# hbb1/2d-gaussian-splatting

Measured on AMD Instinct MI355X. Metric: train iters/sec (full iteration: rasterizer fwd+bwd, L1+SSIM, normal+dist regularisers, Adam) + fwd Msplats/s @1080p, higher is better.
Workload: dtype f32; 1 GPU; garden: trained synthetic capture, 5400000 initial points -> 2136144 surfels after 2500 iterations of the reference schedule, 32 views of 1600x1060; steady-state iteration, every loss term on; P=2136144, image=1600x1060, n_pass=6, tiles=6700

## Files before the change

2d-gaussian-splatting_amd/csrc/surfel_api.hip:

```cpp
#include <cstring>
#include <mutex>
#include <string>
#include <vector>

#include <hip/hip_runtime.h>

#include "../../include/surfel_debug.h"
#include "surfel_common.h"
#include "surfel_kernels.h"
#include "train_kernels.h"

using namespace surfel;

namespace {

const char* kStageNames[] = {"preprocess_fwd", "depth_sort_scan", "emit_instances", "tile_sort", "tile_ranges", "blend_fwd",
                             "zero_grec", "blend_bwd", "preprocess_bwd", "knn", "tile_depth_sort"};
enum Stage { ST_PRE = 0, ST_SCAN, ST_EMIT, ST_SORT, ST_RANGES, ST_BLEND, ST_ZERO, ST_BBWD, ST_PBWD, ST_KNN, ST_TSORT, ST_COUNT };
static_assert(sizeof(kStageNames) / sizeof(kStageNames[0]) == ST_COUNT, "one name per stage");

struct CapEntry {
    int W = 0, H = 0; int64_t maxR = -1; unsigned frames = 0; int uniform_streak = 0; int boost = 0; unsigned last_overflow = 0;
    int slot() const; void begin_frame(); int64_t capacity(int end_bit) const; void record_count(int64_t R, bool overflowed);
};
// ... 43 lines not shown
    template <typename T> T* take(size_t count) {
        off = align_up(off);
        T* p = base ? reinterpret_cast<T*>(base + off) : nullptr;
        off += count * sizeof(T);
        return p;
    }
    size_t size() const { return align_up(off); }
};

struct GeomState {
    float* rec; float* depths; uint32_t* tiles_touched; uint8_t* clamped;
    uint32_t *dkey_a, *dkey_b, *ord_a, *ord_b;
    uint32_t* offsets;
    uint32_t* rects;
    float* shjac;
    char* temp;
    static GeomState carve(void* base, int P, size_t temp_bytes, size_t* total) {
        Carver c(base); GeomState g;
        g.rec = c.take<float>((size_t)P * REC_F);
        g.depths = c.take<float>(P);
        g.tiles_touched = c.take<uint32_t>(P);
        g.clamped = c.take<uint8_t>(P);
        g.dkey_a = c.take<uint32_t>(P); g.dkey_b = c.take<uint32_t>(P);
        g.ord_a = c.take<uint32_t>(P); g.ord_b = c.take<uint32_t>(P);
        g.offsets = c.take<uint32_t>(P);
        g.rects = c.take<uint32_t>(P);
        g.shjac = c.take<float>((size_t)9 * P);
        g.temp = c.take<char>(temp_bytes);
        if (total) *total = c.size();
        return g;
    }
};

struct BinState {
    uint32_t* point_list; uint32_t* vals_alt; uint32_t* keys_a; uint32_t* keys_b; char* sort_temp;
    float4* strm_rec = nullptr; uint32_t* strm_mask = nullptr;
    static bool wants_stream(size_t R) { return g_opt_stream != 0 && R > 0 && (long long)R <= STRM_MAX_R; }
    static BinState carve(void* base, size_t R, size_t sort_bytes, size_t* total, bool stream = false) {
        Carver c(base); BinState b;
        b.point_list = c.take<uint32_t>(R);
        b.vals_alt = c.take<uint32_t>(R);
        b.keys_a = c.take<uint32_t>(R);
// ... 204 lines not shown
    tm.begin(); launch_tile_depth_sort(pa.gx * pa.gy, maxR, img.ranges, bin.point_list, geom.dkey_a, bin.vals_alt, bin.keys_a, bin.keys_b, fused_ranges, s);
    STAGE_END(tm, ST_TSORT);
    return 0;
}

int64_t bin_exact(const PreprocessArgs& pa, int end_bit, int per_tile, int64_t R, const GeomState& geom, BinState* bin,
                  const ImgState& img, const uint32_t* hR, hipEvent_t evR, bool stream, surfel_alloc_fn binning_alloc, void* binning_user,
                  StageTimer& tm, hipStream_t s) {
    if (per_tile < 0 && R < 0) {
        HIP_TRY(hipEventSynchronize(evR));
        per_tile = per_tile_pays(pinned_total(hR, false), pa.gx, pa.gy);
    }
    tm.begin();
    const uint32_t* order = geom.ord_a;
    if (!per_tile) {
        const int which = radix_sort_pairs_u32(geom.dkey_a, geom.ord_a, geom.dkey_b, geom.ord_b, (size_t)pa.P, 0, 32, geom.temp, s, true);
        if (which < 0) return fail(SURFEL_E_LIMIT, "too many surfels for the depth sort");
        order = which ? geom.ord_b : geom.ord_a;
    }
    launch_scan_gather(geom.tiles_touched, order, pa.pack_tiles, geom.offsets, (size_t)pa.P, pa.zero_b, s);
    STAGE_END(tm, ST_SCAN);
    if (R < 0) {
        HIP_TRY(hipEventSynchronize(evR));
        R = pinned_total(hR, false);
    }
    if (int e = alloc_bin((size_t)R, radix_sort_scratch_bytes((size_t)R), stream, binning_alloc, binning_user, bin)) return e;
    if (R == 0) return 0;
    const bool odd = radix_sort_result_buffer((size_t)R, 0, end_bit) == 1;
    uint32_t* va = odd ? bin->vals_alt : bin->point_list;
    uint32_t* vb = odd ? bin->point_list : bin->vals_alt;
    tm.begin();
    launch_emit_instances(pa.P, geom.rec, geom.rects, order, pa.pack_tiles ? ((1u << PACK_ID_BITS) - 1u) : 0xffffffffu, geom.offsets, bin->keys_a, va, pa.gx,
                          reinterpret_cast<uint32_t*>(bin->sort_temp), (uint32_t)radix_sort_head_words((size_t)R), s);
    STAGE_END(tm, ST_EMIT);
    tm.begin();
    const int wk = radix_sort_pairs_u32(bin->keys_a, va, bin->keys_b, vb, (size_t)R, 0, end_bit, bin->sort_temp, s, true);
    if (wk < 0) return fail(SURFEL_E_LIMIT, "too many tile instances for the tile sort");
    STAGE_END(tm, ST_SORT);
    tm.begin(); launch_tile_ranges(R, wk ? bin->keys_b : bin->keys_a, img.ranges, s); STAGE_END(tm, ST_RANGES);
    if (per_tile) {
        tm.begin(); launch_tile_depth_sort(pa.gx * pa.gy, R, img.ranges, bin->point_list, geom.dkey_a, bin->vals_alt, bin->keys_a, bin->keys_b, false, s);
        STAGE_END(tm, ST_TSORT);
    }
    return R;
}

int blend(CapEntry* ce, int W, int H, int gx, int gy, const ImgState& img, const void* img_base, const BinState& bin, const float* rec,
          const float* background, float* out_color, float* out_others, int avg_list, bool jac, int tile_order, StageTimer& tm, hipStream_t s) {
    run_tile_order(ce, img.ranges, gx, gy, img.tile_map, img.total + 2 * R_SLOTS + 1, tile_order, s);
    BlendFwdArgs ba{};
    ba.W = W; ba.H = H; ba.gx = gx; ba.gy = gy;
    ba.ranges = img.ranges; ba.point_list = bin.point_list; ba.rec = rec; ba.bg = background;
    ba.out_color = out_color; ba.out_others = out_others; ba.final_T = img.final_T; ba.n_contrib = img.n_contrib;
    ba.tile_map = img.tile_map; ba.map_flag = img.total + 2 * R_SLOTS + 1; ba.map_len = tile_map_len(gx, gy);
// ... 189 lines not shown
        GeomState::carve(nullptr, P, temp_bytes, &geom_bytes);
        void* geom_base = geom_alloc(geom_user, geom_bytes);
        if (!geom_base) return fail(SURFEL_E_ALLOC, "geometry buffer allocation failed");
        geom = GeomState::carve(geom_base, P, temp_bytes, nullptr);

        PreprocessArgs pa{};
        pa.P = P; pa.D = D; pa.M = M; pa.W = width; pa.H = height; pa.gx = gx; pa.gy = gy; pa.scale_modifier = scale_modifier;
        pa.cull = opt_cull;
        pa.pack_tiles = P < (1 << PACK_ID_BITS) ? 1 : 0;
        pa.means3D = means3D; pa.opacities = opacities; pa.scales = scales; pa.rotations = rotations;
        pa.transMat_precomp = transMat_precomp; pa.colors_precomp = colors_precomp; pa.shs = shs;
        pa.viewmatrix = viewmatrix; pa.projmatrix = projmatrix; pa.campos = cam_pos;
        pa.rec = geom.rec; pa.depths = geom.depths; pa.depth_keys = geom.dkey_a; pa.ident = geom.ord_a; pa.radii = radii;
        pa.tiles_touched = geom.tiles_touched; pa.clamped = geom.clamped; pa.total_instances = img.total; pa.rects = geom.rects;
        pa.shjac = jac ? geom.shjac : nullptr;
        pa.zero_a = reinterpret_cast<uint32_t*>(geom.temp); pa.zero_a_words = (uint32_t)radix_sort_head_words((size_t)P);
        pa.zero_b = reinterpret_cast<uint32_t*>(geom.temp + psort_bytes); pa.zero_b_words = (uint32_t)scan_scratch_words((size_t)P);

        const int end_bit = higher_msb((uint32_t)(gx * gy));
        int per_tile = opt_tile_sort == 2 ? 1 : (opt_tile_sort == 0 ? 0 : -1);
        if (per_tile < 0 && g_th.last_R >= 0 && g_th.last_W == width && g_th.last_H == height) per_tile = per_tile_pays(g_th.last_R, gx, gy);
        const int64_t cap = (opt_capacity && per_tile == 1 && debug != 1) ? ce->capacity(end_bit) : 0;
        if (cap > 0) {
            if (int e = alloc_bin((size_t)cap, capacity_sort_scratch_bytes((size_t)cap, end_bit), opt_stream, binning_alloc, binning_user, &bin)) return e;
            pa.zero_c = reinterpret_cast<uint32_t*>(bin.sort_temp); pa.zero_c_words = (uint32_t)bin_emit_head_words();
            pa.block_totals = geom.offsets;
        }
        tm.begin(); launch_preprocess_fwd(pa, s); STAGE_END(tm, ST_PRE);
        uint32_t* hR = pinned_u32();
        hipEvent_t evR = r_event();
// ... 51 lines not shown
    hipStream_t s = static_cast<hipStream_t>(stream);
    if (P == 0) return 0;
    if (!scratch_alloc || !geom_buffer || !binning_buffer || !image_buffer) return fail(SURFEL_E_INVALID, "buffer / allocator is NULL");
    if (!dL_dout_color || !dL_dout_others || !dL_dmeans2D || !dL_dopacity || !dL_dcolors || !dL_dmeans3D)
        return fail(SURFEL_E_INVALID, "gradient pointer is NULL");
    if (transMat_precomp && !dL_dtransMat) return fail(SURFEL_E_INVALID, "dL_dtransMat is NULL but transMat_precomp was given");
    if (!transMat_precomp && (!dL_dscales || !dL_drots || !scales || !rotations)) return fail(SURFEL_E_INVALID, "scale/rotation pointers are NULL");
    const int gx = (width + TILE - 1) / TILE, gy = (height + TILE - 1) / TILE;

    GeomState geom = GeomState::carve(const_cast<void*>(geom_buffer), P, 0, nullptr);
    BinState bin = BinState::carve(const_cast<void*>(binning_buffer), (size_t)R, 0, nullptr);
    ImgState img = ImgState::carve(const_cast<void*>(image_buffer), width, height, nullptr);

    const size_t grec_bytes = align_up((size_t)(R > 0 ? R : 1) * GREC_F * sizeof(float));
    const size_t cut_bytes = align_up((size_t)gx * gy * sizeof(uint2));
    float* grec = static_cast<float*>(scratch_alloc(scratch_user, grec_bytes + cut_bytes + (size_t)P));
    if (!grec) return fail(SURFEL_E_ALLOC, "gradient record allocation failed");
    const bool use_cut = (debug_in & SURFEL_OPT_TILE_CUTS) ? true : ((debug_in & SURFEL_OPT_ZERO_RECORDS) ? false : R >= ((int64_t)1 << 21));
    uint2* cut = use_cut ? reinterpret_cast<uint2*>(reinterpret_cast<char*>(grec) + grec_bytes) : nullptr;
    uint8_t* has_rec = use_cut ? reinterpret_cast<uint8_t*>(grec) + grec_bytes + cut_bytes : nullptr;
    if (has_rec) HIP_TRY(hipMemsetAsync(has_rec, 0, (size_t)P, s));
    StageTimer tm(debug, s);

    BlendBwdArgs bb{};
    bb.W = width; bb.H = height; bb.gx = gx; bb.gy = gy;
    bb.ranges = img.ranges; bb.point_list = bin.point_list; bb.rec = geom.rec; bb.bg = background;
    bb.final_T = img.final_T; bb.n_contrib = img.n_contrib; bb.dL_dpix = dL_dout_color; bb.dL_dothers = dL_dout_others;
    bb.tile_map = img.tile_map; bb.map_flag = img.total + 2 * R_SLOTS + 1; bb.map_len = tile_map_len(gx, gy);
    bb.grec = grec; bb.cut = cut; bb.has_rec = has_rec; bb.depths = geom.depths; bb.variant = opt_variant; bb.stats = g_blend_stats; bb.walk_word = img.total + 2 * R_SLOTS + 2;
    bool have_jac = false;
    {
        const float4* srec = nullptr; const uint32_t* smask = nullptr;
        const bool found = stream_lookup(binning_buffer, image_buffer, &srec, &smask, &have_jac);
        if (found && !(debug_in & SURFEL_OPT_BWD_GATHER) && g_opt_stream) { bb.strm_rec = srec; bb.strm_mask = smask; }
    }
    bb.n_dev = img.total + 2 * R_SLOTS; bb.n_cap = (uint32_t)(R < 0xffffffffll ? R : 0xffffffffll);
// ... 57 lines not shown
```

2d-gaussian-splatting_amd/csrc/surfel_kernels.h:

```cpp
#pragma once
#include <hip/hip_runtime.h>
#include <stdint.h>

namespace surfel {

struct PreprocessArgs {
    int P, D, M, W, H, gx, gy;
    int cull;
    int pack_tiles;
    float scale_modifier;
    const float* means3D; const float* opacities; const float* scales; const float* rotations;
    const float* transMat_precomp; const float* colors_precomp; const float* shs;
    const float* viewmatrix; const float* projmatrix; const float* campos;
    float* rec; float* depths; uint32_t* depth_keys; uint32_t* ident; int* radii; uint32_t* tiles_touched; uint8_t* clamped;
    uint32_t* rects;
    float* shjac;
    uint32_t* total_instances;
    uint32_t* block_totals;
    uint32_t* zero_a; uint32_t zero_a_words;
    uint32_t* zero_b; uint32_t zero_b_words;
    uint32_t* zero_c; uint32_t zero_c_words;
};

struct BlendFwdArgs {
    int W, H, gx, gy;
    const uint2* ranges; const uint32_t* point_list; const float* rec; const float* bg;
    float* out_color; float* out_others; float* final_T; uint32_t* n_contrib;
    const int* tile_map; const uint32_t* map_flag; int map_len;
    unsigned long long* stats;
    int avg_list;
    float4* strm_rec; uint32_t* strm_mask;
    const uint32_t* totals; uint32_t* walk_word;
};

struct BlendBwdArgs {
    int W, H, gx, gy;
// ... 37 lines not shown
void launch_tile_order(const uint2* ranges, int gx, int gy, int* map, uint32_t* map_flag , int force, uint32_t* verdict, hipStream_t s);
void launch_blend_fwd(const BlendFwdArgs& a, hipStream_t s);
bool launch_blend_fwd_writes_stream(const BlendFwdArgs& a);
void set_fwd_pipe(int v);
void launch_mark_visible(int P, const float* means3D, const float* vm, uint8_t* present, hipStream_t s);
void launch_blend_bwd(const BlendBwdArgs& a, hipStream_t s);
void launch_blend_bwd_scan(const BlendBwdArgs& a, hipStream_t s);
void launch_preprocess_bwd(const PreprocessBwdArgs& a, hipStream_t s);
void launch_colour_gradients(const PreprocessBwdArgs& a, hipStream_t s);
void launch_knn(int P, const float* points, float* out, void* scratch, size_t scratch_bytes, hipStream_t s);
size_t knn_scratch_bytes(int P);
size_t radix_sort_scratch_bytes(size_t n);
void set_large_sort_impl(int v);
int radix_sort_passes(size_t n, int begin_bit, int end_bit);
int radix_sort_result_buffer(size_t n, int begin_bit, int end_bit);
int radix_sort_pairs_u32(uint32_t* keys_a, uint32_t* vals_a, uint32_t* keys_b, uint32_t* vals_b, size_t n, int begin_bit, int end_bit,
                         void* scratch, hipStream_t s, bool head_zeroed = false);
size_t radix_sort_head_words(size_t n);
size_t scan_scratch_words(size_t n);
void launch_tile_depth_sort(int ntiles, int64_t R, uint2* ranges, uint32_t* point_list, const uint32_t* depth_keys, uint32_t* tmp_ids,
                            uint32_t* tmp_keys, uint32_t* tmp_rank, bool decode, hipStream_t s);
void launch_scan_gather(const uint32_t* vals, const uint32_t* order, int packed, uint32_t* out, size_t n, void* zeroed_scratch, hipStream_t s);
bool capacity_binning_ok(size_t cap, int end_bit);
size_t capacity_sort_scratch_bytes(size_t cap, int end_bit);
size_t bin_emit_head_words();
void launch_bin_emit(int P, const uint32_t* tiles_touched, const uint32_t* rects, const uint32_t* block_totals, float* rec, uint32_t* keys, uint32_t* vals,
                     int gx, size_t cap, void* sort_scratch , int end_bit, uint32_t* n_out, uint32_t* n_host ,
                     hipStream_t s);
int radix_sort_pairs_u32_devn(uint32_t* keys_a, uint32_t* vals_a, uint32_t* keys_b, uint32_t* vals_b, size_t cap, int end_bit, const uint32_t* n_dev,
                              void* scratch, uint2* ranges, hipStream_t s);
void launch_tile_ranges_devn(size_t cap, const uint32_t* n_dev, const uint32_t* keys, uint2* ranges, hipStream_t s);

// ... 2 lines not shown
```

2d-gaussian-splatting_amd/csrc/surfel_preprocess.hip:

```cpp
#include "surfel_common.h"
#include "surfel_kernels.h"

namespace surfel {


__device__ __constant__ float SH_C0 = 0.28209479177387814f;
__device__ __constant__ float SH_C1 = 0.4886025119029199f;
__device__ __constant__ float SH_C2[5] = {1.0925484305920792f, -1.0925484305920792f, 0.31539156525252005f,
                                          -1.0925484305920792f, 0.5462742152960396f};
__device__ __constant__ float SH_C3[7] = {-0.5900435899266435f, 2.890611442640554f, -0.4570457994644658f,
                                          0.3731763325901154f, -0.4570457994644658f, 1.445305721320277f,
                                          -0.5900435899266435f};

__device__ __forceinline__ void sh_basis_gradient(int D, float x, float y, float z, float (&Bx)[16], float (&By)[16], float (&Bz)[16]) {
#pragma unroll
    for (int k = 0; k < 16; k++) { Bx[k] = 0.f; By[k] = 0.f; Bz[k] = 0.f; }
    if (D > 0) {
        By[1] = -SH_C1; Bz[2] = SH_C1; Bx[3] = -SH_C1;
        if (D > 1) {
            const float xx = x * x, yy = y * y, zz = z * z, xy = x * y, yz = y * z, xz = x * z;
            Bx[4] = SH_C2[0] * y; By[4] = SH_C2[0] * x;
            By[5] = SH_C2[1] * z; Bz[5] = SH_C2[1] * y;
            Bx[6] = SH_C2[2] * -2.f * x; By[6] = SH_C2[2] * -2.f * y; Bz[6] = SH_C2[2] * 4.f * z;
            Bx[7] = SH_C2[3] * z; Bz[7] = SH_C2[3] * x;
// ... 259 lines not shown
        const int wave = threadIdx.x >> 6, lane = threadIdx.x & 63;
        const int first = blockIdx.x * 256 + wave * 64;
        const int npieces = 12 * min(64, a.P - first);
        const float4* __restrict__ src = reinterpret_cast<const float4*>(a.shs) + (size_t)first * 12;
        const unsigned base = __builtin_amdgcn_readfirstlane(lds_offset(&s_sh[wave][0]));
#pragma unroll
        for (int v = 0; v < 12; v++) {
            const int p = v * 64 + lane;
            if (p < npieces) dma16(src + p, base + (unsigned)v * 1024u);
        }
        sh_lds = &s_sh[wave][lane * 12];
    }
    for (uint32_t w = (uint32_t)i; w < a.zero_a_words; w += gridDim.x * blockDim.x) a.zero_a[w] = 0u;
    for (uint32_t w = (uint32_t)i; w < a.zero_b_words; w += gridDim.x * blockDim.x) a.zero_b[w] = 0u;
    for (uint32_t w = (uint32_t)i; w < a.zero_c_words; w += gridDim.x * blockDim.x) a.zero_c[w] = 0u;
    uint32_t tiles = i < a.P ? preprocess_one(a, i, sh_lds) : 0u;
    const uint32_t vis = (uint32_t)__popcll(__ballot(tiles != 0u));
#pragma unroll
    for (int o = 32; o > 0; o >>= 1) tiles += __shfl_xor(tiles, o);
    if ((threadIdx.x & 63) == 0) { s_tot[threadIdx.x >> 6] = tiles; s_vis[threadIdx.x >> 6] = vis; }
    __syncthreads();
    if (threadIdx.x == 0) {
        const uint32_t t = s_tot[0] + s_tot[1] + s_tot[2] + s_tot[3];
        if (a.block_totals) a.block_totals[blockIdx.x] = t;
        if (t) {
            atomicAdd(a.total_instances + (blockIdx.x % R_SLOTS), t);
            atomicAdd(a.total_instances + R_SLOTS + (blockIdx.x % R_SLOTS), s_vis[0] + s_vis[1] + s_vis[2] + s_vis[3]);
        }
    }
}
// ... 649 lines not shown
```

2d-gaussian-splatting_amd/csrc/surfel_sort.hip:

```cpp
#include <hip/hip_runtime.h>
#include <stdint.h>

#include <cstring>
#include <rocprim/device/device_radix_sort.hpp>

#include "surfel_common.h"
#include "surfel_kernels.h"

namespace surfel {

constexpr size_t RS_ONESWEEP_MAX_ITEMS = (size_t)1 << 20;
constexpr size_t g_onesweep_max = RS_ONESWEEP_MAX_ITEMS;
int g_large_sort_impl = 2;
void set_large_sort_impl(int v) { g_large_sort_impl = v < 0 ? 0 : (v > 3 ? 2 : v); }
static inline bool use_rocprim(size_t n, int begin_bit, int end_bit) {
    if (begin_bit != 0) return false;
    if (g_large_sort_impl == 3) return true;
    if (n <= g_onesweep_max) return false;
    if (g_large_sort_impl != 2) return g_large_sort_impl == 1;
    return n > ((size_t)1 << 25);
}
static size_t rocprim_sort_temp_bytes(size_t n) {
    thread_local size_t last_n = 0, last_bytes = 0;
    if (n == last_n && last_bytes) return last_bytes;
// ... 2 lines not shown
    (void)rocprim::radix_sort_pairs(nullptr, bytes, nul, nul, nul, nul, n, 0u, 32u, (hipStream_t)0);
    last_n = n; last_bytes = bytes;
    return bytes;
}

constexpr int RS_THREADS = 256;
constexpr int RS_IPT = 8;
constexpr int RS_TILE = RS_THREADS * RS_IPT;
static inline bool rs_onesweep(size_t n) { return n <= g_onesweep_max; }
constexpr int RS_BITS = 8;
constexpr int RS_RADIX = 1 << RS_BITS;
constexpr int RS_MAX_PASSES = 4;
constexpr uint32_t ST_AGG = 1u << 30, ST_PREFIX = 2u << 30, ST_VALUE = (1u << 30) - 1u;

constexpr size_t RS_HEAD_WORDS = RS_MAX_PASSES * RS_RADIX + 64;

static inline uint32_t rs_nblocks(size_t n) { return (uint32_t)((n + RS_TILE - 1) / RS_TILE); }

size_t radix_sort_scratch_bytes(size_t n) {
    if (!rs_onesweep(n)) {
        const size_t own = ((size_t)RS_RADIX * rs_nblocks(n) + RS_RADIX) * sizeof(uint32_t) + 256;
        const size_t rp = rocprim_sort_temp_bytes(n) + 256;
        return own > rp ? own : rp;
    }
    const size_t own = (RS_HEAD_WORDS + (size_t)RS_MAX_PASSES * rs_nblocks(n) * RS_RADIX) * sizeof(uint32_t) + 256;
    const size_t rp = g_large_sort_impl == 3 ? rocprim_sort_temp_bytes(n) + 256 : 0;
    return own > rp ? own : rp;
}
int radix_sort_passes(size_t, int begin_bit, int end_bit) { return (end_bit - begin_bit + RS_BITS - 1) / RS_BITS; }
int radix_sort_result_buffer(size_t n, int begin_bit, int end_bit) {
    if (n == 0 || end_bit <= begin_bit) return 0;
    if (use_rocprim(n, begin_bit, end_bit)) return 1;
    return radix_sort_passes(n, begin_bit, end_bit) & 1;
}
size_t radix_sort_head_bytes() { return RS_HEAD_WORDS * sizeof(uint32_t); }

// ... 60 lines not shown
        __syncthreads();
        uint32_t woff = 0;
        for (int w = 0; w < wave; w++) woff += s_w[w];
        const uint32_t carry = s_carry;
        if (i < nblocks) row[i] = carry + woff + x - v;
        __syncthreads();
        if (threadIdx.x == RS_THREADS - 1) s_carry = carry + woff + x;
        __syncthreads();
    }
    if (threadIdx.x == 0) total[blockIdx.x] = s_carry;
}

constexpr int FT_THREADS = 1024, FT_IPT = 4, FT_TILE = FT_THREADS * FT_IPT, FT_WAVES = FT_THREADS / 64;
constexpr int FT_LB = 32;
static inline uint32_t ft_nblocks(size_t n) { return (uint32_t)((n + FT_TILE - 1) / FT_TILE); }

template <bool LOOKBACK, int IPT>
__global__ void __launch_bounds__(FT_THREADS) os_pass_fat_kernel(const uint32_t* __restrict__ keys, const uint32_t* __restrict__ vals,
                                                                 uint32_t* __restrict__ keys_out, uint32_t* __restrict__ vals_out, uint32_t n,
                                                                 int shift, uint32_t mask, const uint32_t* __restrict__ ghist,
                                                                 uint32_t* __restrict__ status, uint32_t* __restrict__ ticket,
                                                                 const uint32_t* __restrict__ n_dev, int hstride, uint2* __restrict__ ranges,
                                                                 uint32_t nblocks) {
    __shared__ uint32_t s_cnt[FT_WAVES][RS_RADIX];
    constexpr int TILE_ITEMS = FT_THREADS * IPT;
    __shared__ uint2 s_item[TILE_ITEMS];
    __shared__ uint32_t s_gbase[RS_RADIX];
    __shared__ uint32_t s_w[4][2];
    __shared__ uint32_t s_tile;
    const int lane = threadIdx.x & 63, wave = threadIdx.x >> 6;
    const uint32_t d_t = threadIdx.x;
    if (LOOKBACK && threadIdx.x == 0) s_tile = atomicAdd(ticket, 1u);
    for (int i = threadIdx.x; i < FT_WAVES * RS_RADIX; i += FT_THREADS) (&s_cnt[0][0])[i] = 0u;
    __syncthreads();
    const uint32_t tile = LOOKBACK ? s_tile : blockIdx.x;
    if (n_dev) n = min(n, *n_dev);
    if (tile * (uint32_t)TILE_ITEMS >= n) return;
    const uint32_t wbase = tile * (uint32_t)TILE_ITEMS + wave * (64 * IPT);
    uint32_t k[IPT], v[IPT], rank[IPT];
#pragma unroll
    for (int it = 0; it < IPT; it++) {
        const uint32_t e = wbase + it * 64 + lane;
        const bool valid = e < n;
        k[it] = valid ? keys[e] : 0xffffffffu;
// ... 74 lines not shown
    for (int it = 0; it < IPT; it++) {
        const uint32_t e = wbase + it * 64 + lane;
        if (e < n) {
            const uint32_t d = (k[it] >> shift) & mask;
            s_item[s_cnt[wave][d] + rank[it]] = make_uint2(k[it], v[it]);
        }
    }
    __syncthreads();
    const uint32_t items = min((uint32_t)TILE_ITEMS, n - tile * (uint32_t)TILE_ITEMS);
#pragma unroll
    for (int it = 0; it < IPT; it++) {
        const uint32_t q = (uint32_t)it * FT_THREADS + threadIdx.x;
        if (q < items) {
            const uint2 kv = s_item[q];
            const uint32_t dst = s_gbase[(kv.x >> shift) & mask] + q;
            keys_out[dst] = kv.x;
            vals_out[dst] = kv.y;
            if (ranges) {
                const bool first = q == 0u || s_item[q - 1].x != kv.x;
                const bool last = q + 1u == items || s_item[q + 1].x != kv.x;
                if (first) atomicMax(&ranges[kv.x].x, ~dst);
                if (last) atomicMax(&ranges[kv.x].y, dst + 1u);
            }
        }
    }
}

size_t radix_sort_head_words(size_t n) { return rs_onesweep(n) ? RS_HEAD_WORDS : 0; }

constexpr int SC_IPT = 8, SC_TILE = RS_THREADS * SC_IPT;
size_t scan_scratch_words(size_t n) { return 64 + (n + SC_TILE - 1) / SC_TILE; }

__global__ void __launch_bounds__(RS_THREADS) scan_gather_kernel(const uint32_t* __restrict__ vals, const uint32_t* __restrict__ order, int packed,
                                                                 uint32_t* __restrict__ out, uint32_t n, uint32_t* __restrict__ scratch) {
    __shared__ uint32_t s_w[4];
    __shared__ uint32_t s_tile, s_excl;
    uint32_t* ticket = scratch;
    uint32_t* status = scratch + 64;
    const int lane = threadIdx.x & 63, wave = threadIdx.x >> 6;
    if (threadIdx.x == 0) s_tile = atomicAdd(ticket, 1u);
    __syncthreads();
    const uint32_t tile = s_tile;
    const uint32_t base = tile * SC_TILE + threadIdx.x * SC_IPT;
    uint32_t v[SC_IPT], sum = 0;
#pragma unroll
    for (int i = 0; i < SC_IPT; i++) {
        const uint32_t e = base + i;
        uint32_t t = 0u;
        if (e < n) {
            const uint32_t ov = order[e];
            if (packed) { t = ov >> PACK_ID_BITS; if (t == PACK_TILES_MAX) t = vals[ov & ((1u << PACK_ID_BITS) - 1u)]; }
            else t = vals[ov];
        }
        v[i] = t;
        sum += v[i];
    }
    uint32_t x = sum;
#pragma unroll
    for (int o = 1; o < 64; o <<= 1) { const uint32_t y = __shfl_up(x, o); if (lane >= o) x += y; }
    if (lane == 63) s_w[wave] = x;
    __syncthreads();
    uint32_t woff = 0;
    for (int w = 0; w < wave; w++) woff += s_w[w];
    const uint32_t agg = s_w[0] + s_w[1] + s_w[2] + s_w[3];
    if (wave == 0) {
        uint32_t excl = 0;
        if (tile == 0) {
            if (lane == 0) st_agent(status, agg | ST_PREFIX);
        } else {
            if (lane == 0) st_agent(status + tile, agg | ST_AGG);
            int p = (int)tile - 1;
            for (;;) {
                const int idx = p - lane;
                const uint32_t sw = idx >= 0 ? ld_agent(status + idx) : ST_PREFIX;
                const unsigned long long ready = __ballot((sw >> 30) != 0u);
                const unsigned long long pref = __ballot((sw & ST_PREFIX) != 0u);
                const int nready = ready == ~0ull ? 64 : __builtin_ctzll(~ready);
                const int firstp = pref ? __builtin_ctzll(pref) : 64;
                const int take = min(nready, firstp + 1);
// ... 8 lines not shown
            if (lane == 0) st_agent(status + tile, (excl + agg) | ST_PREFIX);
        }
        if (lane == 0) s_excl = excl;
    }
    __syncthreads();
    uint32_t run = s_excl + woff + x - sum;
#pragma unroll
    for (int i = 0; i < SC_IPT; i++) {
        run += v[i];
        if (base + i < n) out[base + i] = run;
    }
}

void launch_scan_gather(const uint32_t* vals, const uint32_t* order, int packed, uint32_t* out, size_t n, void* zeroed_scratch, hipStream_t s) {
    if (n == 0) return;
    hipLaunchKernelGGL(scan_gather_kernel, dim3((unsigned)((n + SC_TILE - 1) / SC_TILE)), dim3(RS_THREADS), 0, s, vals, order, packed, out, (uint32_t)n,
                       static_cast<uint32_t*>(zeroed_scratch));
}


template <int E>
__device__ __forceinline__ void tile_sort_regs(uint32_t n, uint32_t* __restrict__ pl, const uint32_t* __restrict__ depth_keys,
                                               unsigned long long* __restrict__ s, uint32_t tid) {
    unsigned long long v[E];
#pragma unroll
    for (int e = 0; e < E; e++) {
        const uint32_t idx = (uint32_t)e * RS_THREADS + tid;
        v[e] = ~0ull;
        if (idx < n) { const uint32_t id = pl[idx]; v[e] = ((unsigned long long)depth_keys[id] << 32) | id; }
    }
#pragma unroll
// ... 82 lines not shown
    for (uint32_t i = tid; i < n; i += RS_THREADS) pl[rank[i]] = ids[i];
}

void launch_tile_depth_sort(int ntiles, int64_t R, uint2* ranges, uint32_t* point_list, const uint32_t* depth_keys, uint32_t* tmp_ids,
                            uint32_t* tmp_keys, uint32_t* tmp_rank, bool decode, hipStream_t st) {
    if (ntiles <= 0) return;
    if (R <= (int64_t)256 * ntiles)
        hipLaunchKernelGGL(tile_depth_sort_kernel<2048>, dim3(ntiles), dim3(RS_THREADS), 0, st, ranges, point_list, depth_keys, tmp_ids, tmp_keys,
                           tmp_rank, decode ? 1 : 0);
    else
        hipLaunchKernelGGL(tile_depth_sort_kernel<4096>, dim3(ntiles), dim3(RS_THREADS), 0, st, ranges, point_list, depth_keys, tmp_ids, tmp_keys,
                           tmp_rank, decode ? 1 : 0);
}

int radix_sort_pairs_u32(uint32_t* keys_a, uint32_t* vals_a, uint32_t* keys_b, uint32_t* vals_b, size_t n, int begin_bit, int end_bit,
                         void* scratch, hipStream_t s, bool head_zeroed) {
    if (n == 0 || end_bit <= begin_bit) return 0;
    if (n >= ST_VALUE) return -1;
    const uint32_t nblocks = rs_nblocks(n);
    const int passes = radix_sort_passes(n, begin_bit, end_bit);
    if (passes > RS_MAX_PASSES) return -1;
    int cur = 0;
    if (use_rocprim(n, begin_bit, end_bit)) {
        size_t bytes = rocprim_sort_temp_bytes(n);
        if (rocprim::radix_sort_pairs(scratch, bytes, keys_a, keys_b, vals_a, vals_b, n, (unsigned)begin_bit, (unsigned)end_bit, s) != hipSuccess) return -1;
        return 1;
    }
    if (!rs_onesweep(n)) {
        uint32_t* hist = static_cast<uint32_t*>(scratch);
        uint32_t* total = hist + (size_t)RS_RADIX * nblocks;
        for (int p = 0; p < passes; p++) {
            const int bit = begin_bit + p * RS_BITS;
            const int nb = end_bit - bit < RS_BITS ? end_bit - bit : RS_BITS;
            const uint32_t mask = (1u << nb) - 1u;
            const uint32_t* kin = cur ? keys_b : keys_a; const uint32_t* vin = cur ? vals_b : vals_a;
            uint32_t* kout = cur ? keys_a : keys_b; uint32_t* vout = cur ? vals_a : vals_b;
            const uint32_t fb = ft_nblocks(n);
            hipLaunchKernelGGL(rs_hist_fat_kernel<FT_IPT>, dim3(fb), dim3(FTH_THREADS), 0, s, kin, (uint32_t)n, bit, mask, hist, fb);
            hipLaunchKernelGGL(rs_scan_kernel, dim3(RS_RADIX), dim3(RS_THREADS), 0, s, hist, fb, total);
            hipLaunchKernelGGL((os_pass_fat_kernel<false, FT_IPT>), dim3(fb), dim3(FT_THREADS), 0, s, kin, vin, kout, vout, (uint32_t)n, bit, mask, total, hist,
                               (uint32_t*)nullptr, (const uint32_t*)nullptr, 1, (uint2*)nullptr, fb);
            cur ^= 1;
        }
        return cur;
    }
    uint32_t* ghist = static_cast<uint32_t*>(scratch);
    uint32_t* ticket = ghist + RS_MAX_PASSES * RS_RADIX;
    uint32_t* status = ghist + RS_HEAD_WORDS;
    if (!head_zeroed) (void)hipMemsetAsync(scratch, 0, RS_HEAD_WORDS * sizeof(uint32_t), s);
    hipLaunchKernelGGL(os_hist_kernel, dim3(nblocks), dim3(RS_THREADS), 0, s, keys_a, (uint32_t)n, begin_bit, end_bit, passes, ghist, status, nblocks);
    for (int p = 0; p < passes; p++) {
        const int bit = begin_bit + p * RS_BITS;
        const int nb = end_bit - bit < RS_BITS ? end_bit - bit : RS_BITS;
        const uint32_t mask = (1u << nb) - 1u;
        const uint32_t* kin = cur ? keys_b : keys_a; const uint32_t* vin = cur ? vals_b : vals_a;
        uint32_t* kout = cur ? keys_a : keys_b; uint32_t* vout = cur ? vals_a : vals_b;
        hipLaunchKernelGGL((os_pass_fat_kernel<true, FT_IPT>), dim3(ft_nblocks(n)), dim3(FT_THREADS), 0, s, kin, vin, kout, vout, (uint32_t)n, bit, mask,
                           ghist + p * RS_RADIX, status + (size_t)p * nblocks * RS_RADIX, ticket + p, (const uint32_t*)nullptr, 1, (uint2*)nullptr, 0u);
        cur ^= 1;
    }
    return cur;
}

constexpr int BE_HSTRIDE = 32;
size_t bin_emit_head_words() { return (size_t)RS_MAX_PASSES * RS_RADIX * BE_HSTRIDE + 64; }

constexpr int BE_THREADS = 1024;
__global__ void __launch_bounds__(BE_THREADS) bin_emit_kernel(int P, const uint32_t* __restrict__ tiles_touched, const uint32_t* __restrict__ rects,
                                                              const uint32_t* __restrict__ block_totals, uint32_t nblock_totals, float* __restrict__ rec,
                                                              uint32_t* __restrict__ keys, uint32_t* __restrict__ vals, int gx, uint32_t cap,
                                                              uint32_t* __restrict__ ghist, uint32_t* __restrict__ sort_status,
                                                              uint32_t sort_status_words, int passes, int end_bit, uint32_t* __restrict__ n_out,
                                                              uint32_t* __restrict__ n_host) {
// ... 52 lines not shown
                              void* scratch, uint2* ranges, hipStream_t s) {
    const uint32_t nblocks = rs_nblocks(cap);
    const int passes = radix_sort_passes(cap, 0, end_bit);
    uint32_t* ghist = static_cast<uint32_t*>(scratch);
    uint32_t* ticket = ghist + (size_t)RS_MAX_PASSES * RS_RADIX * BE_HSTRIDE;
    uint32_t* status = ghist + bin_emit_head_words();
    int cur = 0;
    for (int p = 0; p < passes; p++) {
        const int bit = p * RS_BITS;
        const int nb = end_bit - bit < RS_BITS ? end_bit - bit : RS_BITS;
        const uint32_t mask = (1u << nb) - 1u;
        const uint32_t* kin = cur ? keys_b : keys_a; const uint32_t* vin = cur ? vals_b : vals_a;
        uint32_t* kout = cur ? keys_a : keys_b; uint32_t* vout = cur ? vals_a : vals_b;
        hipLaunchKernelGGL((os_pass_fat_kernel<true, FT_IPT>), dim3(ft_nblocks(cap)), dim3(FT_THREADS), 0, s, kin, vin, kout, vout, (uint32_t)cap, bit, mask,
                           ghist + (size_t)p * RS_RADIX * BE_HSTRIDE, status + (size_t)p * nblocks * RS_RADIX, ticket + p, n_dev, BE_HSTRIDE,
                           p == passes - 1 ? ranges : (uint2*)nullptr, 0u);
        cur ^= 1;
    }
    return cur;
}
bool capacity_binning_ok(size_t cap, int end_bit) { return rs_onesweep(cap) && radix_sort_passes(cap, 0, end_bit) <= 2 && g_large_sort_impl != 3; }
size_t bin_emit_sort_status_words(size_t cap, int end_bit) { return (size_t)radix_sort_passes(cap, 0, end_bit) * rs_nblocks(cap) * RS_RADIX; }
size_t capacity_sort_scratch_bytes(size_t cap, int end_bit) { return (bin_emit_head_words() + bin_emit_sort_status_words(cap, end_bit)) * sizeof(uint32_t) + 256; }

void launch_bin_emit(int P, const uint32_t* tiles_touched, const uint32_t* rects, const uint32_t* block_totals, float* rec, uint32_t* keys, uint32_t* vals,
                     int gx, size_t cap, void* sort_scratch, int end_bit, uint32_t* n_out, uint32_t* n_host, hipStream_t s) {
    uint32_t* ghist = static_cast<uint32_t*>(sort_scratch);
    hipLaunchKernelGGL(bin_emit_kernel, dim3((unsigned)((P + BE_THREADS - 1) / BE_THREADS)), dim3(BE_THREADS), 0, s, P, tiles_touched, rects, block_totals,
                       (uint32_t)((P + 255) / 256), rec, keys, vals, gx, (uint32_t)cap, ghist, ghist + bin_emit_head_words(), (uint32_t)bin_emit_sort_status_words(cap, end_bit),
                       radix_sort_passes(cap, 0, end_bit), end_bit, n_out, n_host);
}
// ... 3 lines not shown
```

Before: 308.6 train-iters/s.

## Fuse tile-range extraction into final sort pass and skip unread key writes

In the exact binning path the final radix pass now writes tile ranges directly, and the last block fixes them up, so the separate tile_ranges kernel is skipped. The final pass also skips writing sorted keys where no later stage reads them, for both the depth sort and the tile sort. The has_rec flag array moves into the geometry state and is zeroed inside preprocess, replacing a separate memset in backward. The large-sort path can pick 5 items per thread to cut block count, and the scan kernel grows to 1024 threads. In exchange there is extra last-block tail work, one more done-counter atomic, and more template instantiations.

```diff
diff --git a/2d-gaussian-splatting_amd/csrc/surfel_api.hip b/2d-gaussian-splatting_amd/csrc/surfel_api.hip
--- a/2d-gaussian-splatting_amd/csrc/surfel_api.hip
+++ b/2d-gaussian-splatting_amd/csrc/surfel_api.hip
@@ -81,6 +81,7 @@
     uint32_t* offsets;
     uint32_t* rects;
     float* shjac;
+    uint8_t* has_rec;
     char* temp;
     static GeomState carve(void* base, int P, size_t temp_bytes, size_t* total) {
         Carver c(base); GeomState g;
@@ -93,6 +94,7 @@
         g.offsets = c.take<uint32_t>(P);
         g.rects = c.take<uint32_t>(P);
         g.shjac = c.take<float>((size_t)9 * P);
+        g.has_rec = c.take<uint8_t>(P);
         g.temp = c.take<char>(temp_bytes);
         if (total) *total = c.size();
         return g;
@@ -327,7 +329,8 @@
     tm.begin();
     const uint32_t* order = geom.ord_a;
     if (!per_tile) {
-        const int which = radix_sort_pairs_u32(geom.dkey_a, geom.ord_a, geom.dkey_b, geom.ord_b, (size_t)pa.P, 0, 32, geom.temp, s, true);
+        SortTail order_only{}; order_only.keys_unread = true;
+        const int which = radix_sort_pairs_u32(geom.dkey_a, geom.ord_a, geom.dkey_b, geom.ord_b, (size_t)pa.P, 0, 32, geom.temp, s, true, order_only);
         if (which < 0) return fail(SURFEL_E_LIMIT, "too many surfels for the depth sort");
         order = which ? geom.ord_b : geom.ord_a;
     }
@@ -347,10 +350,13 @@
                           reinterpret_cast<uint32_t*>(bin->sort_temp), (uint32_t)radix_sort_head_words((size_t)R), s);
     STAGE_END(tm, ST_EMIT);
     tm.begin();
-    const int wk = radix_sort_pairs_u32(bin->keys_a, va, bin->keys_b, vb, (size_t)R, 0, end_bit, bin->sort_temp, s, true);
+    SortTail tail{};
+    const bool fused_ranges = radix_sort_leaves_ranges((size_t)R, 0, end_bit);
+    if (fused_ranges) { tail.ranges = img.ranges; tail.nranges = (uint32_t)(pa.gx * pa.gy); tail.keys_unread = true; }
+    const int wk = radix_sort_pairs_u32(bin->keys_a, va, bin->keys_b, vb, (size_t)R, 0, end_bit, bin->sort_temp, s, true, tail);
     if (wk < 0) return fail(SURFEL_E_LIMIT, "too many tile instances for the tile sort");
     STAGE_END(tm, ST_SORT);
-    tm.begin(); launch_tile_ranges(R, wk ? bin->keys_b : bin->keys_a, img.ranges, s); STAGE_END(tm, ST_RANGES);
+    if (!fused_ranges) { tm.begin(); launch_tile_ranges(R, wk ? bin->keys_b : bin->keys_a, img.ranges, s); STAGE_END(tm, ST_RANGES); }
     if (per_tile) {
         tm.begin(); launch_tile_depth_sort(pa.gx * pa.gy, R, img.ranges, bin->point_list, geom.dkey_a, bin->vals_alt, bin->keys_a, bin->keys_b, false, s);
         STAGE_END(tm, ST_TSORT);
@@ -570,6 +576,7 @@
         pa.rec = geom.rec; pa.depths = geom.depths; pa.depth_keys = geom.dkey_a; pa.ident = geom.ord_a; pa.radii = radii;
         pa.tiles_touched = geom.tiles_touched; pa.clamped = geom.clamped; pa.total_instances = img.total; pa.rects = geom.rects;
         pa.shjac = jac ? geom.shjac : nullptr;
+        pa.has_rec = geom.has_rec;
         pa.zero_a = reinterpret_cast<uint32_t*>(geom.temp); pa.zero_a_words = (uint32_t)radix_sort_head_words((size_t)P);
         pa.zero_b = reinterpret_cast<uint32_t*>(geom.temp + psort_bytes); pa.zero_b_words = (uint32_t)scan_scratch_words((size_t)P);
 
@@ -651,12 +658,11 @@
 
     const size_t grec_bytes = align_up((size_t)(R > 0 ? R : 1) * GREC_F * sizeof(float));
     const size_t cut_bytes = align_up((size_t)gx * gy * sizeof(uint2));
-    float* grec = static_cast<float*>(scratch_alloc(scratch_user, grec_bytes + cut_bytes + (size_t)P));
+    float* grec = static_cast<float*>(scratch_alloc(scratch_user, grec_bytes + cut_bytes));
     if (!grec) return fail(SURFEL_E_ALLOC, "gradient record allocation failed");
     const bool use_cut = (debug_in & SURFEL_OPT_TILE_CUTS) ? true : ((debug_in & SURFEL_OPT_ZERO_RECORDS) ? false : R >= ((int64_t)1 << 21));
     uint2* cut = use_cut ? reinterpret_cast<uint2*>(reinterpret_cast<char*>(grec) + grec_bytes) : nullptr;
-    uint8_t* has_rec = use_cut ? reinterpret_cast<uint8_t*>(grec) + grec_bytes + cut_bytes : nullptr;
-    if (has_rec) HIP_TRY(hipMemsetAsync(has_rec, 0, (size_t)P, s));
+    uint8_t* has_rec = use_cut ? geom.has_rec : nullptr;
     StageTimer tm(debug, s);
 
     BlendBwdArgs bb{};
diff --git a/2d-gaussian-splatting_amd/csrc/surfel_kernels.h b/2d-gaussian-splatting_amd/csrc/surfel_kernels.h
--- a/2d-gaussian-splatting_amd/csrc/surfel_kernels.h
+++ b/2d-gaussian-splatting_amd/csrc/surfel_kernels.h
@@ -20,6 +20,7 @@
     uint32_t* zero_a; uint32_t zero_a_words;
     uint32_t* zero_b; uint32_t zero_b_words;
     uint32_t* zero_c; uint32_t zero_c_words;
+    uint8_t* has_rec;
 };
 
 struct BlendFwdArgs {
@@ -87,8 +88,13 @@
 void set_large_sort_impl(int v);
 int radix_sort_passes(size_t n, int begin_bit, int end_bit);
 int radix_sort_result_buffer(size_t n, int begin_bit, int end_bit);
+struct SortTail {
+    uint2* ranges = nullptr; uint32_t nranges = 0;
+    bool keys_unread = false;
+};
+bool radix_sort_leaves_ranges(size_t n, int begin_bit, int end_bit);
 int radix_sort_pairs_u32(uint32_t* keys_a, uint32_t* vals_a, uint32_t* keys_b, uint32_t* vals_b, size_t n, int begin_bit, int end_bit,
-                         void* scratch, hipStream_t s, bool head_zeroed = false);
+                         void* scratch, hipStream_t s, bool head_zeroed = false, SortTail tail = SortTail{});
 size_t radix_sort_head_words(size_t n);
 size_t scan_scratch_words(size_t n);
 void launch_tile_depth_sort(int ntiles, int64_t R, uint2* ranges, uint32_t* point_list, const uint32_t* depth_keys, uint32_t* tmp_ids,
diff --git a/2d-gaussian-splatting_amd/csrc/surfel_preprocess.hip b/2d-gaussian-splatting_amd/csrc/surfel_preprocess.hip
--- a/2d-gaussian-splatting_amd/csrc/surfel_preprocess.hip
+++ b/2d-gaussian-splatting_amd/csrc/surfel_preprocess.hip
@@ -297,6 +297,7 @@
     for (uint32_t w = (uint32_t)i; w < a.zero_a_words; w += gridDim.x * blockDim.x) a.zero_a[w] = 0u;
     for (uint32_t w = (uint32_t)i; w < a.zero_b_words; w += gridDim.x * blockDim.x) a.zero_b[w] = 0u;
     for (uint32_t w = (uint32_t)i; w < a.zero_c_words; w += gridDim.x * blockDim.x) a.zero_c[w] = 0u;
+    if (i < a.P) a.has_rec[i] = 0;
     uint32_t tiles = i < a.P ? preprocess_one(a, i, sh_lds) : 0u;
     const uint32_t vis = (uint32_t)__popcll(__ballot(tiles != 0u));
 #pragma unroll
diff --git a/2d-gaussian-splatting_amd/csrc/surfel_sort.hip b/2d-gaussian-splatting_amd/csrc/surfel_sort.hip
--- a/2d-gaussian-splatting_amd/csrc/surfel_sort.hip
+++ b/2d-gaussian-splatting_amd/csrc/surfel_sort.hip
@@ -40,12 +40,14 @@
 constexpr uint32_t ST_AGG = 1u << 30, ST_PREFIX = 2u << 30, ST_VALUE = (1u << 30) - 1u;
 
 constexpr size_t RS_HEAD_WORDS = RS_MAX_PASSES * RS_RADIX + 64;
+constexpr int RS_DONE_WORD = RS_MAX_PASSES * RS_RADIX + 8;
+constexpr size_t RS_LARGE_HEAD_WORDS = 64;
 
 static inline uint32_t rs_nblocks(size_t n) { return (uint32_t)((n + RS_TILE - 1) / RS_TILE); }
 
 size_t radix_sort_scratch_bytes(size_t n) {
     if (!rs_onesweep(n)) {
-        const size_t own = ((size_t)RS_RADIX * rs_nblocks(n) + RS_RADIX) * sizeof(uint32_t) + 256;
+        const size_t own = (RS_LARGE_HEAD_WORDS + (size_t)RS_RADIX * rs_nblocks(n) + RS_RADIX) * sizeof(uint32_t) + 256;
         const size_t rp = rocprim_sort_temp_bytes(n) + 256;
         return own > rp ? own : rp;
     }
@@ -136,6 +138,11 @@
 constexpr int FT_THREADS = 1024, FT_IPT = 4, FT_TILE = FT_THREADS * FT_IPT, FT_WAVES = FT_THREADS / 64;
 constexpr int FT_LB = 32;
 static inline uint32_t ft_nblocks(size_t n) { return (uint32_t)((n + FT_TILE - 1) / FT_TILE); }
+constexpr int FT_IPT_WIDE = 5, FT_SLOTS = 512;
+static inline int large_ipt(size_t n) {
+    const size_t b4 = (n + FT_TILE - 1) / FT_TILE, b5 = (n + FT_THREADS * FT_IPT_WIDE - 1) / (FT_THREADS * FT_IPT_WIDE);
+    return (b5 + FT_SLOTS - 1) / FT_SLOTS < (b4 + FT_SLOTS - 1) / FT_SLOTS ? FT_IPT_WIDE : FT_IPT;
+}
 
 template <bool LOOKBACK, int IPT>
 __global__ void __launch_bounds__(FT_THREADS) os_pass_fat_kernel(const uint32_t* __restrict__ keys, const uint32_t* __restrict__ vals,
@@ -143,13 +150,13 @@
                                                                  int shift, uint32_t mask, const uint32_t* __restrict__ ghist,
                                                                  uint32_t* __restrict__ status, uint32_t* __restrict__ ticket,
                                                                  const uint32_t* __restrict__ n_dev, int hstride, uint2* __restrict__ ranges,
-                                                                 uint32_t nblocks) {
+                                                                 uint32_t nblocks, uint32_t* __restrict__ done, uint32_t nranges) {
     __shared__ uint32_t s_cnt[FT_WAVES][RS_RADIX];
     constexpr int TILE_ITEMS = FT_THREADS * IPT;
     __shared__ uint2 s_item[TILE_ITEMS];
     __shared__ uint32_t s_gbase[RS_RADIX];
     __shared__ uint32_t s_w[4][2];
-    __shared__ uint32_t s_tile;
+    __shared__ uint32_t s_tile, s_done;
     const int lane = threadIdx.x & 63, wave = threadIdx.x >> 6;
     const uint32_t d_t = threadIdx.x;
     if (LOOKBACK && threadIdx.x == 0) s_tile = atomicAdd(ticket, 1u);
@@ -254,7 +261,7 @@
         if (q < items) {
             const uint2 kv = s_item[q];
             const uint32_t dst = s_gbase[(kv.x >> shift) & mask] + q;
-            keys_out[dst] = kv.x;
+            if (keys_out) keys_out[dst] = kv.x;
             vals_out[dst] = kv.y;
             if (ranges) {
                 const bool first = q == 0u || s_item[q - 1].x != kv.x;
@@ -264,16 +271,38 @@
             }
         }
     }
-}
-
-size_t radix_sort_head_words(size_t n) { return rs_onesweep(n) ? RS_HEAD_WORDS : 0; }
-
-constexpr int SC_IPT = 8, SC_TILE = RS_THREADS * SC_IPT;
+    if (done) {
+        __syncthreads();
+        if (threadIdx.x == 0) s_done = atomicAdd(done, 1u);
+        __syncthreads();
+        if (s_done != gridDim.x - 1u) return;
+        for (uint32_t t0 = 0; t0 < nranges; t0 += (uint32_t)FT_THREADS * 8u) {
+            unsigned long long w[8];
+#pragma unroll
+            for (int j = 0; j < 8; j++) {
+                const uint32_t t = t0 + (uint32_t)j * FT_THREADS + threadIdx.x;
+                w[j] = t < nranges ? __hip_atomic_load(reinterpret_cast<const unsigned long long*>(ranges + t), __ATOMIC_RELAXED, __HIP_MEMORY_SCOPE_AGENT) : 0ull;
+            }
+#pragma unroll
+            for (int j = 0; j < 8; j++) {
+                const uint32_t t = t0 + (uint32_t)j * FT_THREADS + threadIdx.x;
+                if ((w[j] >> 32) != 0ull) st_agent(&ranges[t].x, ~(uint32_t)w[j]);
+            }
+        }
+    }
+}
+
+size_t radix_sort_head_words(size_t n) { return rs_onesweep(n) ? RS_HEAD_WORDS : RS_LARGE_HEAD_WORDS; }
+bool radix_sort_leaves_ranges(size_t n, int begin_bit, int end_bit) {
+    return n > 0 && n < ST_VALUE && end_bit > begin_bit && radix_sort_passes(n, begin_bit, end_bit) <= RS_MAX_PASSES && !use_rocprim(n, begin_bit, end_bit);
+}
+
+constexpr int SC_THREADS = 1024, SC_WAVES = SC_THREADS / 64, SC_IPT = 8, SC_TILE = SC_THREADS * SC_IPT;
 size_t scan_scratch_words(size_t n) { return 64 + (n + SC_TILE - 1) / SC_TILE; }
 
-__global__ void __launch_bounds__(RS_THREADS) scan_gather_kernel(const uint32_t* __restrict__ vals, const uint32_t* __restrict__ order, int packed,
+__global__ void __launch_bounds__(SC_THREADS) scan_gather_kernel(const uint32_t* __restrict__ vals, const uint32_t* __restrict__ order, int packed,
                                                                  uint32_t* __restrict__ out, uint32_t n, uint32_t* __restrict__ scratch) {
-    __shared__ uint32_t s_w[4];
+    __shared__ uint32_t s_w[SC_WAVES];
     __shared__ uint32_t s_tile, s_excl;
     uint32_t* ticket = scratch;
     uint32_t* status = scratch + 64;
@@ -300,9 +329,9 @@
     for (int o = 1; o < 64; o <<= 1) { const uint32_t y = __shfl_up(x, o); if (lane >= o) x += y; }
     if (lane == 63) s_w[wave] = x;
     __syncthreads();
-    uint32_t woff = 0;
-    for (int w = 0; w < wave; w++) woff += s_w[w];
-    const uint32_t agg = s_w[0] + s_w[1] + s_w[2] + s_w[3];
+    uint32_t woff = 0, agg = 0;
+#pragma unroll
+    for (int w = 0; w < SC_WAVES; w++) { if (w < wave) woff += s_w[w]; agg += s_w[w]; }
     if (wave == 0) {
         uint32_t excl = 0;
         if (tile == 0) {
@@ -341,7 +370,7 @@
 
 void launch_scan_gather(const uint32_t* vals, const uint32_t* order, int packed, uint32_t* out, size_t n, void* zeroed_scratch, hipStream_t s) {
     if (n == 0) return;
-    hipLaunchKernelGGL(scan_gather_kernel, dim3((unsigned)((n + SC_TILE - 1) / SC_TILE)), dim3(RS_THREADS), 0, s, vals, order, packed, out, (uint32_t)n,
+    hipLaunchKernelGGL(scan_gather_kernel, dim3((unsigned)((n + SC_TILE - 1) / SC_TILE)), dim3(SC_THREADS), 0, s, vals, order, packed, out, (uint32_t)n,
                        static_cast<uint32_t*>(zeroed_scratch));
 }
 
@@ -454,7 +483,7 @@
 }
 
 int radix_sort_pairs_u32(uint32_t* keys_a, uint32_t* vals_a, uint32_t* keys_b, uint32_t* vals_b, size_t n, int begin_bit, int end_bit,
-                         void* scratch, hipStream_t s, bool head_zeroed) {
+                         void* scratch, hipStream_t s, bool head_zeroed, SortTail tail) {
     if (n == 0 || end_bit <= begin_bit) return 0;
     if (n >= ST_VALUE) return -1;
     const uint32_t nblocks = rs_nblocks(n);
@@ -467,19 +496,29 @@
         return 1;
     }
     if (!rs_onesweep(n)) {
-        uint32_t* hist = static_cast<uint32_t*>(scratch);
+        uint32_t* done = static_cast<uint32_t*>(scratch);
+        uint32_t* hist = done + RS_LARGE_HEAD_WORDS;
         uint32_t* total = hist + (size_t)RS_RADIX * nblocks;
+        if (!head_zeroed && tail.ranges) (void)hipMemsetAsync(scratch, 0, RS_LARGE_HEAD_WORDS * sizeof(uint32_t), s);
         for (int p = 0; p < passes; p++) {
+            const bool lastp = p == passes - 1;
             const int bit = begin_bit + p * RS_BITS;
             const int nb = end_bit - bit < RS_BITS ? end_bit - bit : RS_BITS;
             const uint32_t mask = (1u << nb) - 1u;
             const uint32_t* kin = cur ? keys_b : keys_a; const uint32_t* vin = cur ? vals_b : vals_a;
             uint32_t* kout = cur ? keys_a : keys_b; uint32_t* vout = cur ? vals_a : vals_b;
-            const uint32_t fb = ft_nblocks(n);
-            hipLaunchKernelGGL(rs_hist_fat_kernel<FT_IPT>, dim3(fb), dim3(FTH_THREADS), 0, s, kin, (uint32_t)n, bit, mask, hist, fb);
+            const bool wide = large_ipt(n) == FT_IPT_WIDE;
+            const uint32_t fb = wide ? (uint32_t)((n + FT_THREADS * FT_IPT_WIDE - 1) / (FT_THREADS * FT_IPT_WIDE)) : ft_nblocks(n);
+            uint32_t* const ko = lastp && tail.keys_unread ? (uint32_t*)nullptr : kout;
+            uint2* const rg = lastp ? tail.ranges : (uint2*)nullptr;
+            uint32_t* const dn = lastp && tail.ranges ? done : (uint32_t*)nullptr;
+            if (wide) hipLaunchKernelGGL(rs_hist_fat_kernel<FT_IPT_WIDE>, dim3(fb), dim3(FTH_THREADS), 0, s, kin, (uint32_t)n, bit, mask, hist, fb);
+            else hipLaunchKernelGGL(rs_hist_fat_kernel<FT_IPT>, dim3(fb), dim3(FTH_THREADS), 0, s, kin, (uint32_t)n, bit, mask, hist, fb);
             hipLaunchKernelGGL(rs_scan_kernel, dim3(RS_RADIX), dim3(RS_THREADS), 0, s, hist, fb, total);
-            hipLaunchKernelGGL((os_pass_fat_kernel<false, FT_IPT>), dim3(fb), dim3(FT_THREADS), 0, s, kin, vin, kout, vout, (uint32_t)n, bit, mask, total, hist,
-                               (uint32_t*)nullptr, (const uint32_t*)nullptr, 1, (uint2*)nullptr, fb);
+            if (wide) hipLaunchKernelGGL((os_pass_fat_kernel<false, FT_IPT_WIDE>), dim3(fb), dim3(FT_THREADS), 0, s, kin, vin, ko, vout, (uint32_t)n, bit, mask, total, hist,
+                                         (uint32_t*)nullptr, (const uint32_t*)nullptr, 1, rg, fb, dn, tail.nranges);
+            else hipLaunchKernelGGL((os_pass_fat_kernel<false, FT_IPT>), dim3(fb), dim3(FT_THREADS), 0, s, kin, vin, ko, vout, (uint32_t)n, bit, mask, total, hist,
+                                    (uint32_t*)nullptr, (const uint32_t*)nullptr, 1, rg, fb, dn, tail.nranges);
             cur ^= 1;
         }
         return cur;
@@ -493,10 +532,12 @@
         const int bit = begin_bit + p * RS_BITS;
         const int nb = end_bit - bit < RS_BITS ? end_bit - bit : RS_BITS;
         const uint32_t mask = (1u << nb) - 1u;
+        const bool lastp = p == passes - 1;
         const uint32_t* kin = cur ? keys_b : keys_a; const uint32_t* vin = cur ? vals_b : vals_a;
         uint32_t* kout = cur ? keys_a : keys_b; uint32_t* vout = cur ? vals_a : vals_b;
-        hipLaunchKernelGGL((os_pass_fat_kernel<true, FT_IPT>), dim3(ft_nblocks(n)), dim3(FT_THREADS), 0, s, kin, vin, kout, vout, (uint32_t)n, bit, mask,
-                           ghist + p * RS_RADIX, status + (size_t)p * nblocks * RS_RADIX, ticket + p, (const uint32_t*)nullptr, 1, (uint2*)nullptr, 0u);
+        hipLaunchKernelGGL((os_pass_fat_kernel<true, FT_IPT>), dim3(ft_nblocks(n)), dim3(FT_THREADS), 0, s, kin, vin, lastp && tail.keys_unread ? (uint32_t*)nullptr : kout,
+                           vout, (uint32_t)n, bit, mask, ghist + p * RS_RADIX, status + (size_t)p * nblocks * RS_RADIX, ticket + p, (const uint32_t*)nullptr, 1,
+                           lastp ? tail.ranges : (uint2*)nullptr, 0u, lastp && tail.ranges ? ghist + RS_DONE_WORD : (uint32_t*)nullptr, tail.nranges);
         cur ^= 1;
     }
     return cur;
@@ -579,7 +620,7 @@
         uint32_t* kout = cur ? keys_a : keys_b; uint32_t* vout = cur ? vals_a : vals_b;
         hipLaunchKernelGGL((os_pass_fat_kernel<true, FT_IPT>), dim3(ft_nblocks(cap)), dim3(FT_THREADS), 0, s, kin, vin, kout, vout, (uint32_t)cap, bit, mask,
                            ghist + (size_t)p * RS_RADIX * BE_HSTRIDE, status + (size_t)p * nblocks * RS_RADIX, ticket + p, n_dev, BE_HSTRIDE,
-                           p == passes - 1 ? ranges : (uint2*)nullptr, 0u);
+                           p == passes - 1 ? ranges : (uint2*)nullptr, 0u, (uint32_t*)nullptr, 0u);
         cur ^= 1;
     }
     return cur;
```

Result: faster. 311.8 train-iters/s (median of 6 runs) (+1.0%).
